# facebookresearch/seamless_communication

Measured on AMD Instinct MI355X. Metric: S2ST utterances/sec (and real-time factor), seamlessM4T_v2_large, 10 s audio, higher is better.
Workload: dtype f32 activations x f16 weights, f32 accumulate

## Files before the change

include/seamless_hip_internal.h:

```cpp
#ifndef SEAMLESS_HIP_INTERNAL_H_
#define SEAMLESS_HIP_INTERNAL_H_

#include "seamless_hip.h"

#ifdef __cplusplus
extern "C" {
#endif

int sc_decoder_step_family(sc_model* m, int rows, int caller);

int sc_op_knob(const char* name, int dflt);

int sc_op_force_general_gemm(int on);
int sc_op_single_plane(int on);
int sc_op_layernorm(const float* d_x, const float* d_gamma, const float* d_beta, float* d_y, int32_t rows, int32_t C,
                    int32_t act);
int sc_op_linear(const float* d_x, const void* d_w_f16, const float* d_bias, const float* d_res, float* d_y,
                 int32_t M, int32_t N, int32_t K, int32_t act, float alpha, int32_t split, int32_t force_gemv);
int sc_op_skinny_linear(const float* d_x, const void* d_w_f16, const float* d_bias, const float* d_res, float* d_y,
                        int32_t M, int32_t N, int32_t K, int32_t act, float alpha);
int sc_op_skinny_res_ln(const float* d_in, const void* d_w_f16, const float* d_bias, float* d_x_inout,
                        const float* d_gamma, const float* d_beta, float* d_h, int32_t M, int32_t N, int32_t K,
                        int32_t splits);
int sc_op_skinny_argmax(const float* d_x, const void* d_w_f16, int32_t M, int32_t N, int32_t K, int32_t step,
// ... 5 lines not shown
int sc_op_dstep_linear_planes(const float* d_x, const void* d_w_f16, const float* d_bias, float* d_y, int32_t M, int32_t N, int32_t K,
                              int32_t act);
int sc_op_dstep_argmax(const float* d_x, const void* d_w_f16, int32_t M, int32_t N, int32_t K, int32_t step,
                       int32_t min_step_for_eos, int32_t force_eos_step, int32_t pad_idx, int32_t eos_idx, int32_t unk_idx,
                       float unk_penalty, int32_t ntl, int32_t* d_idx, float* d_lprob);
int sc_op_dstep_attention(const float* d_proj, int32_t S, const float* d_bias, float* d_kcache, float* d_vcache, int32_t cap,
                          int32_t pos, const int32_t* d_lens, int32_t cross, int32_t nb, int32_t heads, float* d_out);
int sc_op_dstep3_gemv(int32_t mode, const float* d_x, const void* d_w_f16, const float* d_bias, const float* d_gamma,
                      const float* d_beta, const float* d_res, float* d_y, float* d_h, int32_t M, int32_t N, int32_t K, int32_t act,
                      int32_t rg, int32_t shape);
int sc_op_dstep3_argmax(const float* d_x, const void* d_w_f16, int32_t M, int32_t N, int32_t K, int32_t step,
                        int32_t min_step_for_eos, int32_t force_eos_step, int32_t pad_idx, int32_t eos_idx, int32_t unk_idx,
                        float unk_penalty, int32_t* d_idx, float* d_lprob);
int sc_op_chain_bench(int32_t kind, int32_t rows, int32_t n, int32_t reps, float* us_per_kernel);
int sc_op_conv1d(const float* d_x, const void* d_w_f16_packed, const float* d_bias, const float* d_res, float* d_y,
                 int32_t nb, int32_t t_in, int32_t cin, int32_t cout, int32_t k, int32_t stride, int32_t pad,
                 int32_t dil, const int32_t* d_in_lens, int32_t in_act, int32_t act);
int sc_op_pack_conv_weight(const void* d_w_f16, void* d_dst_f16, int32_t cout, int32_t cin, int32_t k);
int sc_op_conv_transpose1d(const float* d_x, const void* d_v_f16, const void* d_g_f16, const float* d_bias,
                           float* d_y, int32_t nb, int32_t t_in, int32_t cin, int32_t cout, int32_t k,
                           int32_t stride, int32_t pad, int32_t in_act);
int sc_op_linear_presplit(const float* d_x, const void* d_w_f16, const float* d_bias, const float* d_res, float* d_y,
                          void* d_yh_f16, void* d_yl_f16, int32_t M, int32_t N, int32_t K, int32_t act, float alpha);
int sc_op_linear_presplit_argmax(const float* d_x, const void* d_w_f16, const float* d_bias, int32_t* d_idx, int32_t M, int32_t N,
                                 int32_t K);
int sc_op_conv1d_presplit(const float* d_x, const void* d_w_f16_packed, const float* d_bias, const float* d_res, float* d_y,
                          void* d_yh_f16, void* d_yl_f16, int32_t nb, int32_t t, int32_t cin, int32_t cout, int32_t k, int32_t pad,
                          int32_t dil, const unsigned char* d_row_valid, int32_t act);
int sc_op_resblock_pair_ps(const float* d_x, const void* d_w1_packed, const float* d_b1, const void* d_w2_packed, const float* d_b2,
                           float* d_out, int32_t nb, int32_t T, int32_t C, int32_t k, int32_t dil);
int sc_op_resblock_pair(const float* d_x, const void* d_w1_packed, const float* d_b1, const void* d_w2_packed,
                        const float* d_b2, float* d_out, int32_t nb, int32_t T, int32_t C, int32_t k, int32_t dil,
                        float slope, const float* d_avg_a, const float* d_avg_b);
int sc_op_mrf_fused(const float* d_x, const void* const* d_w1_packed, const float* const* d_b1, const void* const* d_w2_packed,
                    const float* const* d_b2, float* d_out, int32_t nb, int32_t T, int32_t C, const int32_t* k, const int32_t* dil,
                    float slope);
int sc_op_attention(const float* d_q, const float* d_k, const float* d_v, float* d_out, int32_t nb, int32_t heads,
                    int32_t sq, int32_t skv, int64_t ldq, int64_t ldk, int64_t ldv, int64_t ldo,
                    const int32_t* d_kv_lens, int32_t causal, const float* d_rel_k, int32_t rel_left,
                    int32_t rel_right);
int sc_op_attention_ex(const float* d_q, const float* d_k, const float* d_v, float* d_out, int32_t nb, int32_t heads,
                       int32_t sq, int32_t skv, int64_t ldq, int64_t ldk, int64_t ldv, int64_t ldo,
                       const int32_t* d_kv_lens, int32_t causal, const float* d_rel_k, int32_t rel_left,
                       int32_t rel_right, const int32_t* d_row_off, const float* d_rp_table, int64_t rp_ld,
                       const float* d_q_bias_u, const float* d_q_bias_v, void* d_out_hi, void* d_out_lo, int64_t ldoh);
int sc_op_glu_dwconv(const float* d_x, const float* d_w, float* d_y, int32_t nb, int32_t T, int32_t C, int32_t k,
                     const int32_t* d_lens);
int sc_op_glu_dwconv_ln(const float* d_x, const float* d_w, const float* d_gamma, const float* d_beta, int32_t act, void* d_yh_f16,
                        void* d_yl_f16, int32_t nb, int32_t T, int32_t C, int32_t k, const int32_t* d_lens, int32_t fused);
int sc_op_layernorm2(const float* d_x, const float* d_ga, const float* d_ba, const float* d_gb, const float* d_bb, float* d_y,
                     void* d_yh_f16, void* d_yl_f16, int32_t rows, int32_t C, int32_t fused);
int sc_op_argmax(const float* d_logits, int32_t rows, int32_t V, int32_t* d_idx, float* d_lprob);

#ifdef __cplusplus
}
#endif
#endif
```

seamless_communication_amd/_lib.py:

```python
from __future__ import annotations

import ctypes as C
from pathlib import Path
from typing import Optional

import os

_VARIANT = os.environ.get("SC_LIB_VARIANT", "")
LIB_PATH = Path(__file__).resolve().parent / (f"libseamless_hip.{_VARIANT}.so" if _VARIANT else "libseamless_hip.so")

SC_ABI_VERSION = 9
SC_MAX_UPSAMPLES = 8
SC_MAX_RESBLOCK_KERNELS = 4
SC_MAX_RESBLOCK_DILATIONS = 4
SC_F16, SC_F32, SC_I32 = 0, 1, 2


class SeamlessHipError(RuntimeError):
    pass


class sc_tensor_desc(C.Structure):
    _fields_ = [
        ("name", C.c_char_p),
# ... 106 lines not shown
    "sc_s2st": (C.c_int, [_P, _P, _i, _i, _P, C.POINTER(sc_gen_opts), _P, _i, C.c_float, _P, _P, _P, _i, _P, _P, _i, _P, _P, _P]),
    "sc_prof_enable": (C.c_int, [C.c_int]),
    "sc_prof_reset": (C.c_int, []),
    "sc_prof_report": (C.c_int64, [C.c_char_p, C.c_int64]),
    "sc_text_to_char_seqs": (C.c_int32, [C.c_int32, _P, _P, _P, _P, _P, C.c_int32, C.c_int32, C.c_int32, _P, C.c_int32, C.c_int32,
                                         _P, _P, C.c_int32, _P]),
    "sc_ngram_blocked_tokens": (C.c_int32, [_PI, C.c_int32, C.c_int32, _PI, C.c_int32]),
    "sc_op_knob": (C.c_int, [C.c_char_p, C.c_int]),
    "sc_op_force_general_gemm": (C.c_int, [C.c_int]),
    "sc_op_single_plane": (C.c_int, [C.c_int]),
    "sc_op_layernorm": (C.c_int, [_P, _P, _P, _P, _i, _i, _i]),
    "sc_op_linear": (C.c_int, [_P, _P, _P, _P, _P, _i, _i, _i, _i, C.c_float, _i, _i]),
    "sc_op_skinny_linear": (C.c_int, [_P, _P, _P, _P, _P, _i, _i, _i, _i, C.c_float]),
    "sc_op_skinny_res_ln": (C.c_int, [_P, _P, _P, _P, _P, _P, _P, _i, _i, _i, _i]),
    "sc_op_skinny_argmax": (C.c_int, [_P, _P, _i, _i, _i, _i, _i, _i, _i, _i, _i, C.c_float, _P, _P]),
    "sc_op_dstep_res_ln": (C.c_int, [_P, _P, _P, _P, _P, _P, _P, _i, _i, _i, _i]),
    "sc_op_dstep_linear_planes": (C.c_int, [_P, _P, _P, _P, _i, _i, _i, _i]),
    "sc_op_dstep_argmax": (C.c_int, [_P, _P, _i, _i, _i, _i, _i, _i, _i, _i, _i, C.c_float, _i, _P, _P]),
    "sc_op_resblock_pair_ps": (C.c_int, [_P, _P, _P, _P, _P, _P, _i, _i, _i, _i, _i]),
    "sc_op_glu_dwconv_ln": (C.c_int, [_P, _P, _P, _P, _i, _P, _P, _i, _i, _i, _i, _P, _i]),
    "sc_op_layernorm2": (C.c_int, [_P, _P, _P, _P, _P, _P, _P, _P, _i, _i, _i]),
    "sc_op_dstep3_gemv": (C.c_int, [_i, _P, _P, _P, _P, _P, _P, _P, _P, _i, _i, _i, _i, _i, _i]),
    "sc_op_dstep3_argmax": (C.c_int, [_P, _P, _i, _i, _i, _i, _i, _i, _i, _i, _i, C.c_float, _P, _P]),
    "sc_op_chain_bench": (C.c_int, [_i, _i, _i, _i, _P]),
    "sc_op_dstep_attention": (C.c_int, [_P, _i, _P, _P, _P, _i, _i, _P, _i, _i, _i, _P]),
    "sc_op_conv1d": (C.c_int, [_P, _P, _P, _P, _P, _i, _i, _i, _i, _i, _i, _i, _i, _P, _i, _i]),
    "sc_op_pack_conv_weight": (C.c_int, [_P, _P, _i, _i, _i]),
    "sc_op_conv_transpose1d": (C.c_int, [_P, _P, _P, _P, _P, _i, _i, _i, _i, _i, _i, _i, _i]),
    "sc_op_linear_presplit": (C.c_int, [_P, _P, _P, _P, _P, _P, _P, _i, _i, _i, _i, C.c_float]),
    "sc_op_linear_presplit_argmax": (C.c_int, [_P, _P, _P, _P, _i, _i, _i]),
    "sc_op_conv1d_presplit": (C.c_int, [_P, _P, _P, _P, _P, _P, _P, _i, _i, _i, _i, _i, _i, _i, _P, _i]),
    "sc_op_mrf_fused": (C.c_int, [_P, _P, _P, _P, _P, _P, _i, _i, _i, _P, _P, C.c_float]),
    "sc_op_resblock_pair": (C.c_int, [_P, _P, _P, _P, _P, _P, _i, _i, _i, _i, _i, C.c_float, _P, _P]),
    "sc_op_attention": (C.c_int, [_P, _P, _P, _P, _i, _i, _i, _i, C.c_int64, C.c_int64, C.c_int64, C.c_int64, _P, _i,
                                  _P, _i, _i]),
    "sc_op_attention_ex": (C.c_int, [_P, _P, _P, _P, _i, _i, _i, _i, C.c_int64, C.c_int64, C.c_int64, C.c_int64, _P, _i,
                                     _P, _i, _i, _P, _P, C.c_int64, _P, _P, _P, _P, C.c_int64]),
    "sc_op_glu_dwconv": (C.c_int, [_P, _P, _P, _i, _i, _i, _i, _P]),
    "sc_op_argmax": (C.c_int, [_P, _i, _i, _P, _P]),
}

_lib: Optional[C.CDLL] = None


def load_library() -> C.CDLL:
    global _lib
    if _lib is not None:
        return _lib
    if not LIB_PATH.exists():
        raise SeamlessHipError(
            f"{LIB_PATH} is missing: build it with `python -m seamless_communication_amd.build` "
            "(there is no CPU fallback for the HIP path)"
        )
    lib = C.CDLL(str(LIB_PATH))
    for name, (res, args) in SIGNATURES.items():
        fn = getattr(lib, name)
        fn.restype = res
        fn.argtypes = args
    if lib.sc_abi_version() != SC_ABI_VERSION:
        raise SeamlessHipError(f"ABI mismatch: library {lib.sc_abi_version()} vs binding {SC_ABI_VERSION}")
    _lib = lib
    return lib


def check(status: int, what: str) -> None:
    if status != 0:
# ... 54 lines not shown
```

seamless_communication_amd/build.py:

```python
from __future__ import annotations

import hashlib
import os
import subprocess
import sys
from concurrent.futures import ThreadPoolExecutor
from pathlib import Path

CSRC = Path(__file__).resolve().parent / "csrc"
LIB = Path(__file__).resolve().parent / "libseamless_hip.so"
OBJ_DIR = CSRC / "build"
SOURCES = [
    "common.cpp", "prof.hip", "k_gemm.hip", "k_gemm2.hip", "k_gemm_ps.hip", "k_resblock.hip", "k_skinny.hip", "k_dstep.hip", "k_dstep3.hip", "k_norm.hip", "k_attn.hip", "k_fbank.hip", "k_misc.hip", "k_beam.hip", "k_engine.hip",
    "model_load.hip", "model_encoder.hip", "model_decoder.hip", "model_t2u.hip", "engine.hip", "api.hip",
]
FLAGS = ["--offload-arch=gfx950", "-O3", "-std=c++17", "-fPIC", "-Wall", "-Wno-unused-function"]


def _hipcc() -> str:
    for cand in (os.environ.get("HIPCC"), "/opt/rocm/bin/hipcc", "hipcc"):
        if cand and (os.path.sep not in cand or os.path.exists(cand)):
            return cand
    raise RuntimeError("hipcc not found")


def _stamp(src: Path, flags=FLAGS) -> str:
    h = hashlib.sha256()
    h.update(src.read_bytes())
    for hdr in sorted(CSRC.glob("*.h")) + sorted((CSRC.parent.parent / "include").glob("*.h")):
        h.update(hdr.read_bytes())
    h.update(" ".join(flags).encode())
    return h.hexdigest()


def _compile(src_name: str, verbose: bool, obj_dir: Path = OBJ_DIR, flags=FLAGS) -> Path:
    src = CSRC / src_name
    obj = obj_dir / (src_name + ".o")
    stamp = obj_dir / (src_name + ".stamp")
    digest = _stamp(src, flags)
    if obj.exists() and stamp.exists() and stamp.read_text() == digest:
        return obj
    cmd = [_hipcc(), *flags, "-x", "hip", "-c", str(src), "-o", str(obj)]
    if verbose:
        print(" ".join(cmd), flush=True)
    r = subprocess.run(cmd, capture_output=True, text=True)
    if r.returncode != 0:
# ... 40 lines not shown
```

seamless_communication_amd/csrc/api.hip:

```cpp
#include <atomic>
#include <cstring>
#include <map>
#include <mutex>
#include <set>

#include "../../include/seamless_hip_internal.h"
#include "engine.h"
#include "model.h"

using namespace sc;

struct sc_model {
    Model m;
};

struct sc_engine {
    std::unique_ptr<Engine> e;
    int device = 0;
    const void* weights = nullptr;
    std::set<sc_model*> attached;
};

static std::mutex g_attach_mu;
static std::map<Engine*, sc_engine*> g_engine_owner;
// ... 1162 lines not shown
    conv1d_presplit(tmp, xh, xl, c1, nullptr, nullptr, th, tl, nb, T, (k * dil - dil) / 2, dil, nullptr, ACT_NONE, 0, nullptr, 0.1f, one ? 0 : 1);
    conv1d_presplit(tmp, th, tl, c2, d_x, d_out, nullptr, nullptr, nb, T, (k - 1) / 2, 1, nullptr, ACT_NONE, 0, nullptr, 0.1f, one ? 0 : 1);
    SC_HIP(hipStreamSynchronize(g_op_stream));
    SC_API_END
}

int sc_op_resblock_pair(const float* d_x, const void* d_w1_packed, const float* d_b1, const void* d_w2_packed,
                        const float* d_b2, float* d_out, int32_t nb, int32_t T, int32_t C, int32_t k, int32_t dil,
                        float slope, const float* d_avg_a, const float* d_avg_b) {
    SC_API_BEGIN
    SC_CHECK(d_x && d_w1_packed && d_w2_packed && d_out, "sc_op_resblock_pair: null argument");
    ResPairArgs a;
    a.x = d_x;
    a.out = d_out;
    a.w1 = static_cast<const __half*>(d_w1_packed);
    a.w2 = static_cast<const __half*>(d_w2_packed);
    a.ldw1 = a.ldw2 = align_up((int64_t)C * k, 32);
    a.b1 = d_b1;
    a.b2 = d_b2;
    a.nb = nb;
    a.T = T;
    a.C = C;
    a.k = k;
    a.dil = dil;
    a.slope = slope;
    a.avg_a = d_avg_a;
    a.avg_b = d_avg_b;
    a.single = g_op_single.load();
    launch_resblock_pair(a, g_op_stream);
    SC_HIP(hipStreamSynchronize(g_op_stream));
    SC_API_END
}

int sc_op_mrf_fused(const float* d_x, const void* const* d_w1_packed, const float* const* d_b1, const void* const* d_w2_packed,
                    const float* const* d_b2, float* d_out, int32_t nb, int32_t T, int32_t C, const int32_t* k, const int32_t* dil,
                    float slope) {
    SC_API_BEGIN
    SC_CHECK(d_x && d_w1_packed && d_b1 && d_w2_packed && d_b2 && d_out && k && dil, "sc_op_mrf_fused: null argument");
    MrfArgs a;
    a.x = d_x;
    a.out = d_out;
    a.nb = nb;
    a.T = T;
    a.C = C;
    a.slope = slope;
    for (int j = 0; j < 3; ++j) a.k[j] = k[j];
    for (int q = 0; q < 9; ++q) {
        a.dil[q] = dil[q];
        a.w1[q] = static_cast<const __half*>(d_w1_packed[q]);
        a.w2[q] = static_cast<const __half*>(d_w2_packed[q]);
        a.ldw1[q] = a.ldw2[q] = align_up((int64_t)C * k[q / 3], 32);
        a.b1[q] = d_b1[q];
        a.b2[q] = d_b2[q];
    }
    a.single = g_op_single.load();
    launch_mrf_fused(a, g_op_stream);
    SC_HIP(hipStreamSynchronize(g_op_stream));
    SC_API_END
}

int sc_op_attention(const float* d_q, const float* d_k, const float* d_v, float* d_out, int32_t nb, int32_t heads,
                    int32_t sq, int32_t skv, int64_t ldq, int64_t ldk, int64_t ldv, int64_t ldo, const int32_t* d_kv_lens,
                    int32_t causal, const float* d_rel_k, int32_t rel_left, int32_t rel_right) {
    SC_API_BEGIN
    AttnArgs a;
    a.q = d_q;
// ... 110 lines not shown
```

seamless_communication_amd/csrc/common.cpp:

```cpp
#include "common.h"
#include <cstdlib>
#include <cstring>

namespace sc {

static thread_local char g_err[1024] = "";

void set_error(const char* fmt, ...) {
    va_list ap;
    va_start(ap, fmt);
    vsnprintf(g_err, sizeof(g_err), fmt, ap);
    va_end(ap);
}

const char* get_error() { return g_err; }

namespace knob {
namespace {
struct Knob {
    const char* name;
    int kind;
    const char* what;
};
const Knob knob_table[] = {
    {"SC_DEBUG_NUMERICS", 0, "honour the switches that change results"},
    {"SC_DEBUG_FILL", 0, "fill fresh scratch blocks with NaN (tests)"},
    {"SC_SPLIT_MODE", 1, "1: Conformer products on the hi fp16 plane only (precision study)"},
    {"SC_ATTN_F32", 1, "attention on the exact-fp32 matrix instruction (round 1)"},
    {"SC_ATTN_VALU", 1, "attention on the vector ALU (round 1)"},
    {"SC_DECODER_GEN1", 1, "decoder step on the first-generation kernels"},
    {"SC_DECODER_GEN2", 1, "decoder step on the second-generation chain"},
    {"SC_DECODE_STEPWISE", 1, "teacher-forced pass step by step instead of one batched forward"},
    {"SC_VOC_SPLIT", 1, "vocoder ResBlock products on both fp16 planes of their activations again (bit 0 wide stages, bit 2 narrow stages); default: hi plane only"},
    {"SC_GEMM_GENERAL", 0, "general GEMM kernel instead of the fast path"}, {"SC_GEMM_PF2", 0, "GEMM prefetch depth"},
    {"SC_GEMM_GROUP_M", 0, "GEMM workgroup order"}, {"SC_GEMM_TILE", 0, "GEMM tile override"},
    {"SC_PS_ILV", 0, "DMA GEMM: interleaved issue"}, {"SC_PS_HALF", 0, "DMA GEMM: mid-slab barrier"}, {"SC_PS_PP", 0, "0: 8-wave DMA GEMM in lock step instead of alternating load / compute segments"},
    {"SC_PS_TILE", 0, "DMA GEMM: largest tile"}, {"SC_PS_MIN256", 0, "DMA GEMM: tiles needed for 256 x 256"},
    {"SC_PS_MIN128", 0, "DMA GEMM: tiles needed for 128 x 128"},
    {"SC_PRESPLIT", 0, "0: Conformer operands split on the fly"}, {"SC_ENC_FUSE", 0, "0: separate Conformer element-wise launches"},
    {"SC_D3_RG_SMALL", 0, "decoder step: rows per row group, N = 1024 products"}, {"SC_D3_RG_FFN", 0, "decoder step: rows per row group, FFN-in"},
    {"SC_G3_STATIONARY", 0, "row-group products of wide steps: 0 one workgroup per row group, n = workgroup budget of the weight-stationary launch"},
    {"SC_G3_TILES", 0, "0: FFN-out of wide steps on the weight-stationary row-group walk instead of tile-owning waves"},
    {"SC_G3_TOUCH", 0, "weight-stationary products: bit 0 cooperative L2 touch of the activations, bit 1 K slices per XCD (FFN-out); default 3"},
    {"SC_D3_FFN_IN", 0, "decoder step: FFN-in workgroup shape"}, {"SC_D3_FFN_OUT", 0, "decoder step: FFN-out workgroup shape"},
    {"SC_MMA_GRAPH", 0, "streaming decoder step from a captured graph"}, 
    {"SC_T2U_GROUPS", 0, "NAR T2U: length buckets"}, {"SC_T2U_PACKED", 0, "0: NAR decoder on padded buckets"},
    {"SC_T2U_FUSED_ARGMAX", 0, "0: unit logits written out, arg-max as its own launch"},
    {"SC_VOC_PS", 0, "0: vocoder wide stages on the register-staged convolution"}, {"SC_VOC_MRF", 0, "0: narrow vocoder stages as nine pair launches"},
    {"SC_VOC_GROUPS", 0, "vocoder: length buckets"}, {"SC_VOC_GROUP_OVERHEAD", 0, "vocoder: bucket planning overhead rows"},
    {"SC_VOC_STREAMS", 0, "vocoder: side chains"},
    {"SC_ENGINE_RG_SMALL", 0, "decode engine: rows per row group, N = 1024 products"},
    {"SC_BEAM_COMPACT", 2, "0: beam search keeps finished utterances' slots"},
    {"SC_GREEDY_COMPACT", 2, "0: greedy generation keeps finished rows in their slots"}, {"SC_GREEDY_POLL", 2, "steps between looks at the finished flags"},
};
constexpr int N_KNOBS = sizeof(knob_table) / sizeof(knob_table[0]);
struct State {
    bool set[N_KNOBS];
    int val[N_KNOBS];
    bool numerics = false;
};
const State& state() {
    static const State st = [] {
        State s{};
        const char* dn = getenv("SC_DEBUG_NUMERICS");
        s.numerics = dn && atoi(dn) != 0;
        for (int i = 0; i < N_KNOBS; ++i) {
// ... 53 lines not shown
```

seamless_communication_amd/csrc/kernels.h:

```cpp
#pragma once
#include <atomic>

#include "common.h"
#include "prof.h"

namespace sc {

enum Act { ACT_NONE = 0, ACT_RELU = 1, ACT_SILU = 2, ACT_TANH = 3 };
enum InAct { IN_NONE = 0, IN_LRELU_01 = 1, IN_LRELU_001 = 2 };

struct GemmArgs {
    const float* A = nullptr;
    int64_t lda = 0;
    const __half* W = nullptr;
    int64_t ldw = 0;
    int64_t w_phase_stride = 0;
    const float* bias = nullptr;
    const float* res = nullptr;
    int64_t ldr = 0;
    float* C = nullptr;
    int64_t ldc = 0;
    int M = 0;
    int N = 0;
    int K = 0;
// ... 32 lines not shown
    int64_t ldcs = 0;
    int M = 0, N = 0, K = 0;
    int act = ACT_NONE;
    float alpha = 1.0f;
    int split = 1;
    float plane_neg_slope = 1.0f;
    int conv_taps = 0, conv_cin = 0, conv_dil = 1, conv_pad = 0, rows_per_item = 0;
    const unsigned char* row_valid = nullptr;
    const int2* row_pos = nullptr;
    float2* amax = nullptr;
    int amax_ld = 0;
};
void launch_gemm_presplit(const GemmPsArgs& a, hipStream_t s);
int gemm_presplit_amax_chunks(int M, int N);
void launch_amax_finish(const float2* part, int ld, int rows, int* out_idx, hipStream_t s);

struct ResPairArgs {
    const float* x = nullptr;
    float* out = nullptr;
    const __half* w1 = nullptr;
    int64_t ldw1 = 0;
    const float* b1 = nullptr;
    const __half* w2 = nullptr;
    int64_t ldw2 = 0;
    const float* b2 = nullptr;
    int nb = 0, T = 0, C = 0, k = 0, dil = 1;
    float slope = 0.1f;
    const float* avg_a = nullptr;
    const float* avg_b = nullptr;
    int single = 0;
};
bool resblock_pair_supported(int C, int k, int dil);
void launch_resblock_pair(const ResPairArgs& a, hipStream_t s);

struct MrfArgs {
    const float* x = nullptr;
    float* out = nullptr;
    int nb = 0, T = 0, C = 0;
    float slope = 0.1f;
    int halo = 0;
    int k[3] = {0, 0, 0};
    int dil[9] = {1, 1, 1, 1, 1, 1, 1, 1, 1};
    const __half* w1[9] = {};
    const __half* w2[9] = {};
    int64_t ldw1[9] = {};
    int64_t ldw2[9] = {};
    const float* b1[9] = {};
    const float* b2[9] = {};
    int single = 0;
};
bool mrf_fused_supported(int C, const int* k, const int* dil);
void launch_mrf_fused(const MrfArgs& a, hipStream_t s);

void launch_gemv(const float* x, int64_t ldx, const __half* W, int64_t ldw, const float* bias,
                 const float* res, int64_t ldr, float* out, int64_t ldo, int M, int N, int K,
                 int act, float alpha, hipStream_t s);

struct SkinnyArgs {
    const float* A = nullptr;
    int64_t lda = 0;
    const __half* W = nullptr;
    int64_t ldw = 0;
    const float* bias = nullptr;
    const float* res = nullptr;
    int64_t ldr = 0;
    float* C = nullptr;
// ... 396 lines not shown
```

seamless_communication_amd/csrc/model_t2u.hip:

```cpp
#include <cstdlib>

#include "model.h"

namespace sc {

namespace {

void attention_self(Model& m, const float* qkv, int M, float* out, int nb, int S, const int* d_lens) {
    AttnArgs a;
    a.q = qkv;
    a.k = qkv + M;
    a.v = qkv + 2 * M;
    a.out = out;
    a.ldq = a.ldk = a.ldv = 3 * M;
    a.ldo = M;
    a.nb = nb;
    a.heads = m.cfg.num_heads;
    a.Sq = S;
    a.Skv = S;
    a.kv_lens = d_lens;
    launch_attention(a, m.stream);
}

void text_to_char_seqs(const Model& m, const int32_t* text_seqs, int n, int s_text, std::vector<int32_t>& char_lens,
// ... 449 lines not shown
    int ch = c.voc_upsample_initial_channel;
    int t = T;
    Buf<float> x;
    {
        Buf<float> in(m.pp(), (size_t)n * T * (E + Lg + Sp));
        launch_vocoder_embed(d_units, n, T, m.voc_dict, E, m.voc_lang, Lg, d_lang, m.voc_spkr, Sp, d_spkr, in, m.stream);
        x = Buf<float>(m.pp(), (size_t)n * T * ch);
        conv1d(m, in, m.voc_pre, nullptr, x, n, T, 1, 3, 1, nullptr, IN_NONE, ACT_NONE);
    }
    const int nk = c.voc_num_resblock_kernels;
    SC_CHECK(nk == 3, "sc_vocode: %d resblock kernels (only 3 is implemented)", nk);
    static const int voc_split = knob::value("SC_VOC_SPLIT", 0);
    const int voc_single = (voc_split & 1 ? 0 : 1) | (voc_split & 4 ? 0 : 4);
    for (int i = 0; i < c.voc_num_upsamples; ++i) {
        const ConvT& up = m.voc_ups[i];
        const int t2 = t * up.stride;
        ch = up.cout;
        const size_t sz = (size_t)n * t2 * ch;
        Buf<float> y(m.pp(), sz), tmp(m.pp(), sz), ra(m.pp(), sz), rb(m.pp(), sz);
        Buf<float> rout[3] = {Buf<float>(m.pp(), sz), Buf<float>(m.pp(), sz), Buf<float>(m.pp(), sz)};
        conv_transpose1d(m, x, up, y, n, t, IN_LRELU_01);
        bool fused_avg = false;
        x = Buf<float>(m.pp(), sz);
        static const bool voc_ps = knob::value("SC_VOC_PS", 1) != 0;
        bool wide_ps = voc_ps && g_force_general_gemm.load(std::memory_order_relaxed) == 0 && ch >= 128 && ch % 32 == 0 &&
                       (int64_t)n * t2 * ch * 2 < (1ll << 31);
        for (int j = 0; j < nk && wide_ps; ++j) {
            const ResBlock& r = m.voc_res[i * nk + j];
            for (size_t d = 0; d < r.dil.size(); ++d)
                wide_ps = wide_ps && r.convs1[d].cin == ch && r.convs1[d].cout == ch && r.convs2[d].cin == ch && r.convs2[d].cout == ch &&
                          r.convs1[d].kpad == ch * r.convs1[d].k && r.convs2[d].kpad == ch * r.convs2[d].k && (r.convs1[d].k & 1) &&
                          (r.convs2[d].k & 1);
        }
        if (wide_ps) {
            const bool one_plane = (voc_single & 1) != 0;
            Buf<__half> planes(m.pp(), (one_plane ? 3 : 6) * sz);
            __half* py_h = planes.get();
            __half* pt_h = py_h + sz;
            __half* pn_h = pt_h + sz;
            __half* py_l = one_plane ? nullptr : pn_h + sz;
            __half* pt_l = one_plane ? nullptr : py_l + sz;
            __half* pn_l = one_plane ? nullptr : pt_l + sz;
            launch_lrelu_split_f32(y, 0.1f, py_h, py_l, (int64_t)sz, m.stream);
            for (int j = 0; j < nk; ++j) {
                const ResBlock& r = m.voc_res[i * nk + j];
                const float* cur = y;
                const __half *ch_ = py_h, *cl_ = py_l;
                const int nd = (int)r.dil.size();
                for (int d = 0; d < nd; ++d) {
                    const int k = r.convs1[d].k, k2 = r.convs2[d].k;
                    const bool last = d == nd - 1;
                    float* dst = last ? rout[j].get() : ((d & 1) ? rb.get() : ra.get());
                    const int split = one_plane ? 0 : 1;
                    conv1d_presplit(m, ch_, cl_, r.convs1[d], nullptr, nullptr, pt_h, pt_l, n, t2, (k * r.dil[d] - r.dil[d]) / 2, r.dil[d], nullptr,
                                    ACT_NONE, 0, nullptr, 0.1f, split);
                    conv1d_presplit(m, pt_h, pt_l, r.convs2[d], cur, dst, last ? nullptr : pn_h, last ? nullptr : pn_l, n, t2, (k2 - 1) / 2, 1,
                                    nullptr, ACT_NONE, 0, nullptr, 0.1f, split);
                    cur = dst;
                    ch_ = pn_h;
                    cl_ = pn_l;
                }
            }
            launch_avg3(rout[0], rout[1], rout[2], x, (int64_t)sz, m.stream);
            t = t2;
            continue;
        }
        static const bool voc_mrf = knob::value("SC_VOC_MRF", 1) != 0;
// ... 3 lines not shown
            for (int j = 0; j < nk && ok; ++j) {
                const ResBlock& r = m.voc_res[i * nk + j];
                ok = r.dil.size() == 3;
                for (int d = 0; d < 3 && ok; ++d) {
                    const Conv &c1 = r.convs1[d], &c2 = r.convs2[d];
                    ok = c1.k == r.convs1[0].k && c2.k == c1.k && c1.cin == ch && c1.cout == ch && c2.cin == ch && c2.cout == ch;
                    const int q = j * 3 + d;
                    a.dil[q] = r.dil[d];
                    a.w1[q] = c1.w, a.ldw1[q] = c1.kpad, a.b1[q] = c1.b;
                    a.w2[q] = c2.w, a.ldw2[q] = c2.kpad, a.b2[q] = c2.b;
                }
                if (ok) a.k[j] = r.convs1[0].k;
            }
            if (ok && mrf_fused_supported(ch, a.k, a.dil)) {
                a.x = y.get();
                a.out = x.get();
                a.nb = n;
                a.T = t2;
                a.C = ch;
                a.slope = 0.1f;
                a.single = (voc_single & 4) ? 1 : 0;
                launch_mrf_fused(a, m.stream);
                t = t2;
                continue;
            }
        }
        for (int j = 0; j < nk; ++j) {
            const ResBlock& r = m.voc_res[i * nk + j];
            const float* cur = y;
            const int nd = (int)r.dil.size();
            for (int d = 0; d < nd; ++d) {
                const int k = r.convs1[d].k;
                float* dst = (d == nd - 1) ? rout[j].get() : ((d & 1) ? rb.get() : ra.get());
                const bool fuse = g_force_general_gemm.load(std::memory_order_relaxed) == 0 && r.convs2[d].k == k &&
                                  r.convs1[d].cin == ch && r.convs1[d].cout == ch && r.convs2[d].cin == ch &&
                                  r.convs2[d].cout == ch && resblock_pair_supported(ch, k, r.dil[d]);
                if (fuse) {
                    ResPairArgs a;
                    a.x = cur;
                    a.w1 = r.convs1[d].w;
                    a.ldw1 = r.convs1[d].kpad;
                    a.b1 = r.convs1[d].b;
                    a.w2 = r.convs2[d].w;
                    a.ldw2 = r.convs2[d].kpad;
                    a.b2 = r.convs2[d].b;
                    a.nb = n;
                    a.T = t2;
                    a.C = ch;
                    a.k = k;
                    a.dil = r.dil[d];
                    a.slope = 0.1f;
                    a.single = (voc_single & 4) ? 1 : 0;
                    if (j == nk - 1 && d == nd - 1) {
                        a.avg_a = rout[0];
                        a.avg_b = rout[1];
                        dst = x.get();
                        fused_avg = true;
                    }
                    a.out = dst;
                    launch_resblock_pair(a, m.stream);
                } else {
                    conv1d(m, cur, r.convs1[d], nullptr, tmp, n, t2, 1, (k * r.dil[d] - r.dil[d]) / 2, r.dil[d], nullptr,
                           IN_LRELU_01, ACT_NONE);
                    conv1d(m, tmp, r.convs2[d], cur, dst, n, t2, 1, (k - 1) / 2, 1, nullptr, IN_LRELU_01, ACT_NONE);
                }
                cur = dst;
            }
        }
        if (!fused_avg) launch_avg3(rout[0], rout[1], rout[2], x, (int64_t)sz, m.stream);
        t = t2;
    }
    conv1d(m, x, m.voc_post, nullptr, d_wav, n, t, 1, 3, 1, nullptr, IN_LRELU_001, ACT_TANH);
}

int vocoder_halo_units(const Model& m) {
    const sc_config& c = m.cfg;
    double halo = 3.0, rate = 1.0;
    for (int i = 0; i < c.voc_num_upsamples; ++i) {
        const ConvT& up = m.voc_ups[i];
        halo += (double)up.taps / rate;
        rate *= up.stride;
        int widest = 0;
        for (int j = 0; j < c.voc_num_resblock_kernels; ++j) {
            const ResBlock& r = m.voc_res[i * c.voc_num_resblock_kernels + j];
            int reach = 0;
            for (size_t d = 0; d < r.dil.size(); ++d) reach += (r.convs1[d].k - 1) * r.dil[d] / 2 + (r.convs2[d].k - 1) / 2;
            widest = std::max(widest, reach);
        }
        halo += (double)widest / rate;
    }
    halo += 3.0 / rate;
    return (int)halo + 8;
}
// ... 123 lines not shown
```

Measured before the change: 328.1.

## Fuse wide vocoder ResBlock dilation pairs into one DMA-fed MFMA kernel

Adds a kernel for vocoder ResBlock stages with C=128 or 256 that runs both convolutions of a dilation pair in one launch. The input tile with halo is staged as fp16 in LDS, weights stream through a three-stage LDS ring via buffer_load-to-LDS, and the intermediate activation stays in LDS. The final residual add and the three-way branch average are applied in the epilogue. This replaces two DMA GEMM launches per pair plus the fp16 plane splitting, removing the global round trip of the intermediate, at the cost of halo recompute and heavy LDS use that limits occupancy.

```diff
diff --git a/include/seamless_hip_internal.h b/include/seamless_hip_internal.h
--- a/include/seamless_hip_internal.h
+++ b/include/seamless_hip_internal.h
@@ -61,6 +61,9 @@
 int sc_op_resblock_pair(const float* d_x, const void* d_w1_packed, const float* d_b1, const void* d_w2_packed,
                         const float* d_b2, float* d_out, int32_t nb, int32_t T, int32_t C, int32_t k, int32_t dil,
                         float slope, const float* d_avg_a, const float* d_avg_b);
+int sc_op_resblock_pair_wide(const float* d_x, const void* d_w1_packed, const float* d_b1, const void* d_w2_packed, const float* d_b2,
+                             float* d_out, const float* d_avg_a, const float* d_avg_b, int32_t nb, int32_t T, int32_t C, int32_t k,
+                             int32_t dil);
 int sc_op_mrf_fused(const float* d_x, const void* const* d_w1_packed, const float* const* d_b1, const void* const* d_w2_packed,
                     const float* const* d_b2, float* d_out, int32_t nb, int32_t T, int32_t C, const int32_t* k, const int32_t* dil,
                     float slope);
diff --git a/seamless_communication_amd/_lib.py b/seamless_communication_amd/_lib.py
--- a/seamless_communication_amd/_lib.py
+++ b/seamless_communication_amd/_lib.py
@@ -162,6 +162,7 @@
     "sc_op_conv1d_presplit": (C.c_int, [_P, _P, _P, _P, _P, _P, _P, _i, _i, _i, _i, _i, _i, _i, _P, _i]),
     "sc_op_mrf_fused": (C.c_int, [_P, _P, _P, _P, _P, _P, _i, _i, _i, _P, _P, C.c_float]),
     "sc_op_resblock_pair": (C.c_int, [_P, _P, _P, _P, _P, _P, _i, _i, _i, _i, _i, C.c_float, _P, _P]),
+    "sc_op_resblock_pair_wide": (C.c_int, [_P, _P, _P, _P, _P, _P, _P, _P, _i, _i, _i, _i, _i]),
     "sc_op_attention": (C.c_int, [_P, _P, _P, _P, _i, _i, _i, _i, C.c_int64, C.c_int64, C.c_int64, C.c_int64, _P, _i,
                                   _P, _i, _i]),
     "sc_op_attention_ex": (C.c_int, [_P, _P, _P, _P, _i, _i, _i, _i, C.c_int64, C.c_int64, C.c_int64, C.c_int64, _P, _i,
diff --git a/seamless_communication_amd/build.py b/seamless_communication_amd/build.py
--- a/seamless_communication_amd/build.py
+++ b/seamless_communication_amd/build.py
@@ -11,7 +11,7 @@
 LIB = Path(__file__).resolve().parent / "libseamless_hip.so"
 OBJ_DIR = CSRC / "build"
 SOURCES = [
-    "common.cpp", "prof.hip", "k_gemm.hip", "k_gemm2.hip", "k_gemm_ps.hip", "k_resblock.hip", "k_skinny.hip", "k_dstep.hip", "k_dstep3.hip", "k_norm.hip", "k_attn.hip", "k_fbank.hip", "k_misc.hip", "k_beam.hip", "k_engine.hip",
+    "common.cpp", "prof.hip", "k_gemm.hip", "k_gemm2.hip", "k_gemm_ps.hip", "k_resblock.hip", "k_resblock_wide.hip", "k_skinny.hip", "k_dstep.hip", "k_dstep3.hip", "k_norm.hip", "k_attn.hip", "k_fbank.hip", "k_misc.hip", "k_beam.hip", "k_engine.hip",
     "model_load.hip", "model_encoder.hip", "model_decoder.hip", "model_t2u.hip", "engine.hip", "api.hip",
 ]
 FLAGS = ["--offload-arch=gfx950", "-O3", "-std=c++17", "-fPIC", "-Wall", "-Wno-unused-function"]
diff --git a/seamless_communication_amd/csrc/api.hip b/seamless_communication_amd/csrc/api.hip
--- a/seamless_communication_amd/csrc/api.hip
+++ b/seamless_communication_amd/csrc/api.hip
@@ -1218,6 +1218,33 @@
     SC_API_END
 }
 
+int sc_op_resblock_pair_wide(const float* d_x, const void* d_w1_packed, const float* d_b1, const void* d_w2_packed, const float* d_b2,
+                             float* d_out, const float* d_avg_a, const float* d_avg_b, int32_t nb, int32_t T, int32_t C, int32_t k,
+                             int32_t dil) {
+    SC_API_BEGIN
+    SC_CHECK(d_x && d_w1_packed && d_w2_packed && d_out, "sc_op_resblock_pair_wide: null argument");
+    ResPairArgs a;
+    a.x = d_x;
+    a.out = d_out;
+    a.w1 = static_cast<const __half*>(d_w1_packed);
+    a.w2 = static_cast<const __half*>(d_w2_packed);
+    a.ldw1 = a.ldw2 = (int64_t)C * k;
+    a.b1 = d_b1;
+    a.b2 = d_b2;
+    a.nb = nb;
+    a.T = T;
+    a.C = C;
+    a.k = k;
+    a.dil = dil;
+    a.slope = 0.1f;
+    a.avg_a = d_avg_a;
+    a.avg_b = d_avg_b;
+    a.single = 1;
+    launch_resblock_wide(a, g_op_stream);
+    SC_HIP(hipStreamSynchronize(g_op_stream));
+    SC_API_END
+}
+
 int sc_op_mrf_fused(const float* d_x, const void* const* d_w1_packed, const float* const* d_b1, const void* const* d_w2_packed,
                     const float* const* d_b2, float* d_out, int32_t nb, int32_t T, int32_t C, const int32_t* k, const int32_t* dil,
                     float slope) {
diff --git a/seamless_communication_amd/csrc/common.cpp b/seamless_communication_amd/csrc/common.cpp
--- a/seamless_communication_amd/csrc/common.cpp
+++ b/seamless_communication_amd/csrc/common.cpp
@@ -32,6 +32,7 @@
     {"SC_DECODER_GEN2", 1, "decoder step on the second-generation chain"},
     {"SC_DECODE_STEPWISE", 1, "teacher-forced pass step by step instead of one batched forward"},
     {"SC_VOC_SPLIT", 1, "vocoder ResBlock products on both fp16 planes of their activations again (bit 0 wide stages, bit 2 narrow stages); default: hi plane only"},
+    {"SC_VOC_WIDE_PAIR", 1, "0: wide vocoder stages (C = 128 / 256) as two DMA GEMM launches per dilation pair instead of one fused pair kernel"},
     {"SC_GEMM_GENERAL", 0, "general GEMM kernel instead of the fast path"}, {"SC_GEMM_PF2", 0, "GEMM prefetch depth"},
     {"SC_GEMM_GROUP_M", 0, "GEMM workgroup order"}, {"SC_GEMM_TILE", 0, "GEMM tile override"},
     {"SC_PS_ILV", 0, "DMA GEMM: interleaved issue"}, {"SC_PS_HALF", 0, "DMA GEMM: mid-slab barrier"}, {"SC_PS_PP", 0, "0: 8-wave DMA GEMM in lock step instead of alternating load / compute segments"},
diff --git a/seamless_communication_amd/csrc/k_resblock_wide.hip b/seamless_communication_amd/csrc/k_resblock_wide.hip
--- /dev/null
+++ b/seamless_communication_amd/csrc/k_resblock_wide.hip
@@ -0,0 +1,277 @@
+#include <algorithm>
+
+#include "kernels.h"
+
+namespace sc {
+
+namespace {
+
+typedef _Float16 half8_t __attribute__((ext_vector_type(8)));
+typedef _Float16 half4_t __attribute__((ext_vector_type(4)));
+typedef float float16_t __attribute__((ext_vector_type(16)));
+typedef float f32x4_t __attribute__((ext_vector_type(4)));
+typedef int i32x4_t __attribute__((ext_vector_type(4)));
+
+constexpr int RW_M1 = 128;
+constexpr int RW_BK = 32;
+constexpr int RW_STAGES = 3;
+constexpr int RW_LDS_MAX = 160 * 1024;
+#define RW_LDS_PTR(p) ((__attribute__((address_space(3))) void*)(p))
+
+template <int C>
+struct RwCfg {
+    static constexpr int NWAVE = C / 32;
+    static constexpr int WGN = NWAVE / 2;
+    static constexpr int BCH = C / (16 * NWAVE);
+    static_assert(C == 128 || C == 256, "wide pair kernel: C = 128 or 256");
+    static_assert(BCH == 2, "two DMA chunks per wave and slab");
+};
+
+__device__ __forceinline__ float rw_lrelu(float v, float slope) { return fmaxf(v, 0.f) + slope * fminf(v, 0.f); }
+
+__device__ __forceinline__ i32x4_t rw_rsrc(const void* base, uint32_t bytes) {
+    const uint64_t b = reinterpret_cast<uint64_t>(base);
+    i32x4_t r;
+    r[0] = __builtin_amdgcn_readfirstlane((int)(uint32_t)b);
+    r[1] = __builtin_amdgcn_readfirstlane((int)(uint32_t)((b >> 32) & 0xffff));
+    r[2] = __builtin_amdgcn_readfirstlane((int)bytes);
+    r[3] = 0x00020000;
+    return r;
+}
+
+__device__ __forceinline__ int rw_swz(int row, int s) { return row * 64 + ((s ^ ((row >> 2) & 3)) << 4); }
+
+template <int C>
+__global__ __launch_bounds__(C * 2) void resblock_wide_kernel(ResPairArgs p, int tiles, uint32_t w1_bytes, uint32_t w2_bytes) {
+    using Cfg = RwCfg<C>;
+    constexpr int NT = Cfg::NWAVE * 64;
+    constexpr int CS = C + 8;
+    constexpr int VPR = C / 4;
+    constexpr int SLAB_HALFS = C * RW_BK;
+    constexpr int BCH = Cfg::BCH;
+    extern __shared__ __attribute__((aligned(16))) unsigned char rw_smem[];
+    _Float16* const ring = reinterpret_cast<_Float16*>(rw_smem);
+    _Float16* const xs = ring + RW_STAGES * SLAB_HALFS;
+
+    const int k = p.k, dil = p.dil, T = p.T;
+    const int H2 = (k - 1) / 2, H1 = dil * (k - 1) / 2;
+    const int TT = RW_M1 - 2 * H2;
+    const int R0 = RW_M1 + 2 * H1;
+    const int NS = k * C / RW_BK;
+    const int NSL = 2 * NS;
+    const float slope = p.slope;
+
+    const int tid = threadIdx.x, lane = tid & 63;
+    const int wave = __builtin_amdgcn_readfirstlane(tid >> 6);
+    const int wm = wave / Cfg::WGN, wn = wave % Cfg::WGN;
+    const int n = blockIdx.x / tiles;
+    const int t0 = (blockIdx.x - n * tiles) * TT;
+    const float* __restrict__ xn = p.x + (int64_t)n * T * C;
+
+    const i32x4_t rw1 = rw_rsrc(p.w1, w1_bytes);
+    const i32x4_t rw2 = rw_rsrc(p.w2, w2_bytes);
+    uint32_t b_voff1[BCH], b_voff2[BCH];
+#pragma unroll
+    for (int j = 0; j < BCH; ++j) {
+        const int row = 16 * (wave * BCH + j) + (lane >> 2);
+        const int seg = (lane & 3) ^ ((row >> 2) & 3);
+        b_voff1[j] = (uint32_t)((row * p.ldw1 + seg * 8) * 2);
+        b_voff2[j] = (uint32_t)((row * p.ldw2 + seg * 8) * 2);
+    }
+    auto issue = [&](int h) {
+        const bool second = h >= NS;
+        const int soff = (second ? h - NS : h) * (RW_BK * 2);
+        _Float16* const st = ring + (h % RW_STAGES) * SLAB_HALFS;
+#pragma unroll
+        for (int j = 0; j < BCH; ++j) {
+            const uint32_t voff = second ? b_voff2[j] : b_voff1[j];
+            const uint32_t m0 = __builtin_amdgcn_readfirstlane((int)(uint32_t)(uintptr_t)RW_LDS_PTR(st + (wave * BCH + j) * 512));
+            if (second)
+                asm volatile("s_mov_b32 m0, %0\n\tbuffer_load_dwordx4 %1, %2, %3 offen lds" : : "s"(m0), "v"(voff), "s"(rw2), "s"(soff) : "memory");
+            else
+                asm volatile("s_mov_b32 m0, %0\n\tbuffer_load_dwordx4 %1, %2, %3 offen lds" : : "s"(m0), "v"(voff), "s"(rw1), "s"(soff) : "memory");
+        }
+    };
+
+    issue(0);
+    if (NSL > 1) issue(1);
+    float bias1[2], bias2[2];
+#pragma unroll
+    for (int j = 0; j < 2; ++j) {
+        const int col = wn * 64 + j * 32 + (lane & 31);
+        bias1[j] = p.b1 ? p.b1[col] : 0.f;
+        bias2[j] = p.b2 ? p.b2[col] : 0.f;
+    }
+    {
+        constexpr int U = 8;
+        const int total = R0 * VPR;
+        for (int base = tid; base < total; base += NT * U) {
+            f32x4_t v[U];
+#pragma unroll
+            for (int u = 0; u < U; ++u) {
+                const int i = base + u * NT;
+                const int r = i / VPR, c4 = i - r * VPR;
+                const int t = t0 - H2 - H1 + r;
+                v[u] = f32x4_t{0.f, 0.f, 0.f, 0.f};
+                if (i < total && t >= 0 && t < T) v[u] = *reinterpret_cast<const f32x4_t*>(xn + (int64_t)t * C + c4 * 4);
+            }
+#pragma unroll
+            for (int u = 0; u < U; ++u) {
+                const int i = base + u * NT;
+                if (i >= total) continue;
+                const int r = i / VPR, c4 = i - r * VPR;
+#pragma unroll
+                for (int e = 0; e < 4; ++e) v[u][e] = rw_lrelu(v[u][e], slope);
+                *reinterpret_cast<half4_t*>(xs + r * CS + c4 * 4) = __builtin_convertvector(v[u], half4_t);
+            }
+        }
+    }
+    __builtin_amdgcn_s_waitcnt(0x0070);
+
+    const int koff = (lane >> 5) * 8;
+    int a_row[2], b_off[2][2];
+#pragma unroll
+    for (int i = 0; i < 2; ++i) a_row[i] = 64 * wm + 32 * i + (lane & 31);
+#pragma unroll
+    for (int kc = 0; kc < 2; ++kc)
+#pragma unroll
+        for (int j = 0; j < 2; ++j) b_off[j][kc] = rw_swz(wn * 64 + j * 32 + (lane & 31), kc * 2 + (lane >> 5));
+
+    float16_t acc[2][2];
+#pragma unroll
+    for (int i = 0; i < 2; ++i)
+#pragma unroll
+        for (int j = 0; j < 2; ++j)
+#pragma unroll
+            for (int r = 0; r < 16; ++r) acc[i][j][r] = 0.f;
+
+    auto step = [&](int g, int tap_step) {
+        if (g + 1 < NSL) __builtin_amdgcn_s_waitcnt(0x0072);
+        else __builtin_amdgcn_s_waitcnt(0x0070);
+        __builtin_amdgcn_s_barrier();
+        asm volatile("" ::: "memory");
+        const int kk = (g < NS ? g : g - NS) * RW_BK;
+        const int tap = kk / C, c0 = kk - tap * C;
+        const char* const st = reinterpret_cast<const char*>(ring + (g % RW_STAGES) * SLAB_HALFS);
+        half8_t af[2][2], bf[2][2];
+#pragma unroll
+        for (int kc = 0; kc < 2; ++kc) {
+#pragma unroll
+            for (int i = 0; i < 2; ++i)
+                af[kc][i] = *reinterpret_cast<const half8_t*>(xs + (a_row[i] + tap * tap_step) * CS + c0 + kc * 16 + koff);
+#pragma unroll
+            for (int j = 0; j < 2; ++j) bf[kc][j] = *reinterpret_cast<const half8_t*>(st + b_off[j][kc]);
+        }
+        const bool more = g + 2 < NSL;
+        __builtin_amdgcn_sched_barrier(0);
+#pragma unroll
+        for (int kc = 0; kc < 2; ++kc)
+#pragma unroll
+            for (int i = 0; i < 2; ++i)
+#pragma unroll
+                for (int j = 0; j < 2; ++j) {
+                    acc[i][j] = __builtin_amdgcn_mfma_f32_32x32x16_f16(af[kc][i], bf[kc][j], acc[i][j], 0, 0, 0);
+                    if (kc == 0 && i == 0 && j == 1) {
+                        __builtin_amdgcn_sched_barrier(0);
+                        if (more) issue(g + 2);
+                        __builtin_amdgcn_sched_barrier(0);
+                    }
+                }
+        asm volatile("" ::: "memory");
+    };
+
+    for (int g = 0; g < NS; ++g) step(g, dil);
+    __builtin_amdgcn_s_waitcnt(0xC07F);
+    __builtin_amdgcn_s_barrier();
+    asm volatile("" ::: "memory");
+#pragma unroll
+    for (int i = 0; i < 2; ++i)
+#pragma unroll
+        for (int j = 0; j < 2; ++j) {
+            const int col = wn * 64 + j * 32 + (lane & 31);
+#pragma unroll
+            for (int r = 0; r < 16; ++r) {
+                const int row = 64 * wm + 32 * i + (r & 3) + 8 * (r >> 2) + 4 * (lane >> 5);
+                const int t = t0 - H2 + row;
+                const float v = (t >= 0 && t < T) ? rw_lrelu((acc[i][j][r] + bias1[j]) * 1.0f, slope) : 0.f;
+                xs[row * CS + col] = (_Float16)v;
+                acc[i][j][r] = 0.f;
+            }
+        }
+
+    for (int g = NS; g < NSL; ++g) step(g, 1);
+
+    float* __restrict__ outn = p.out + (int64_t)n * T * C;
+    const int64_t nTC = (int64_t)n * T * C;
+#pragma unroll
+    for (int i = 0; i < 2; ++i)
+#pragma unroll
+        for (int j = 0; j < 2; ++j) {
+            const int col = wn * 64 + j * 32 + (lane & 31);
+            float res[16], va[16], vb[16];
+#pragma unroll
+            for (int r = 0; r < 16; ++r) {
+                const int row = 64 * wm + 32 * i + (r & 3) + 8 * (r >> 2) + 4 * (lane >> 5);
+                const int64_t off = (int64_t)min(t0 + row, T - 1) * C + col;
+                res[r] = xn[off];
+                if (p.avg_a) {
+                    va[r] = p.avg_a[nTC + off];
+                    vb[r] = p.avg_b[nTC + off];
+                }
+            }
+#pragma unroll
+            for (int r = 0; r < 16; ++r) {
+                const int row = 64 * wm + 32 * i + (r & 3) + 8 * (r >> 2) + 4 * (lane >> 5);
+                const int t = t0 + row;
+                float v = (acc[i][j][r] + bias2[j]) * 1.0f + res[r];
+                if (p.avg_a) v = ((va[r] + vb[r]) + v) / 3.0f;
+                if (row < TT && t < T) outn[(int64_t)t * C + col] = v;
+            }
+        }
+}
+
+size_t rw_lds_bytes(int C, int k, int dil) {
+    return (size_t)RW_STAGES * C * RW_BK * sizeof(_Float16) + (size_t)(RW_M1 + dil * (k - 1)) * (C + 8) * sizeof(_Float16);
+}
+
+template <int C>
+void launch_rw_cfg(const ResPairArgs& a, hipStream_t s) {
+    static bool attr_set = false;
+    if (!attr_set) {
+        SC_HIP(hipFuncSetAttribute(reinterpret_cast<const void*>(&resblock_wide_kernel<C>), hipFuncAttributeMaxDynamicSharedMemorySize, RW_LDS_MAX));
+        attr_set = true;
+    }
+    const int TT = RW_M1 - (a.k - 1);
+    const int tiles = cdiv(a.T, TT);
+    const size_t lds = rw_lds_bytes(C, a.k, a.dil);
+    char name[48];
+    snprintf(name, sizeof(name), "resblock_wide_c%d", C);
+    const double rows = (double)a.nb * a.T;
+    prof::Scope scope(name, 2.0 * 2.0 * rows * C * (double)C * a.k,
+                      4.0 * rows * C * (a.avg_a ? 4.0 : 2.0) + 2.0 * 2.0 * C * (double)C * a.k, s);
+    hipLaunchKernelGGL((resblock_wide_kernel<C>), dim3((unsigned)(a.nb * tiles)), dim3(RwCfg<C>::NWAVE * 64), lds, s, a, tiles,
+                       (uint32_t)(C * a.ldw1 * 2), (uint32_t)(C * a.ldw2 * 2));
+}
+
+}
+
+bool resblock_wide_supported(int C, int k, int dil) {
+    if (!(C == 128 || C == 256) || k < 1 || (k & 1) == 0 || dil < 1) return false;
+    return RW_M1 - (k - 1) >= 32 && rw_lds_bytes(C, k, dil) <= (size_t)RW_LDS_MAX;
+}
+
+void launch_resblock_wide(const ResPairArgs& a, hipStream_t s) {
+    SC_CHECK(resblock_wide_supported(a.C, a.k, a.dil), "resblock wide pair: unsupported C=%d k=%d dil=%d", a.C, a.k, a.dil);
+    SC_CHECK(a.single, "resblock wide pair: multiplies the hi fp16 plane only");
+    SC_CHECK(a.nb > 0 && a.T > 0 && a.x && a.out && a.w1 && a.w2 && a.x != a.out, "resblock wide pair: empty problem, null operand or in-place call");
+    SC_CHECK(a.ldw1 % 8 == 0 && a.ldw2 % 8 == 0 && a.ldw1 >= (int64_t)a.k * a.C && a.ldw2 >= (int64_t)a.k * a.C &&
+                 (int64_t)a.C * std::max(a.ldw1, a.ldw2) * 2 < (1ll << 31),
+             "resblock wide pair: packed weight rows too short or too long");
+    SC_CHECK((a.avg_a == nullptr) == (a.avg_b == nullptr), "resblock wide pair: avg_a/avg_b must be given together");
+    SC_CHECK((int64_t)a.nb * cdiv(a.T, RW_M1 - (a.k - 1)) < (1ll << 31), "resblock wide pair: grid too large");
+    if (a.C == 128) launch_rw_cfg<128>(a, s);
+    else launch_rw_cfg<256>(a, s);
+    SC_LAUNCH_CHECK();
+}
+
+}
diff --git a/seamless_communication_amd/csrc/kernels.h b/seamless_communication_amd/csrc/kernels.h
--- a/seamless_communication_amd/csrc/kernels.h
+++ b/seamless_communication_amd/csrc/kernels.h
@@ -88,6 +88,8 @@
 };
 bool resblock_pair_supported(int C, int k, int dil);
 void launch_resblock_pair(const ResPairArgs& a, hipStream_t s);
+bool resblock_wide_supported(int C, int k, int dil);
+void launch_resblock_wide(const ResPairArgs& a, hipStream_t s);
 
 struct MrfArgs {
     const float* x = nullptr;
diff --git a/seamless_communication_amd/csrc/model_t2u.hip b/seamless_communication_amd/csrc/model_t2u.hip
--- a/seamless_communication_amd/csrc/model_t2u.hip
+++ b/seamless_communication_amd/csrc/model_t2u.hip
@@ -505,7 +505,15 @@
                           r.convs1[d].kpad == ch * r.convs1[d].k && r.convs2[d].kpad == ch * r.convs2[d].k && (r.convs1[d].k & 1) &&
                           (r.convs2[d].k & 1);
         }
-        if (wide_ps) {
+        static const bool voc_wide_pair = knob::value("SC_VOC_WIDE_PAIR", 1) != 0;
+        bool wide_pair = voc_wide_pair && (voc_single & 1) && g_force_general_gemm.load(std::memory_order_relaxed) == 0;
+        for (int j = 0; j < nk && wide_pair; ++j) {
+            const ResBlock& r = m.voc_res[i * nk + j];
+            for (size_t d = 0; d < r.dil.size(); ++d)
+                wide_pair = wide_pair && r.convs1[d].cin == ch && r.convs1[d].cout == ch && r.convs2[d].cin == ch && r.convs2[d].cout == ch &&
+                            r.convs2[d].k == r.convs1[d].k && resblock_wide_supported(ch, r.convs1[d].k, r.dil[d]);
+        }
+        if (wide_ps && !wide_pair) {
             const bool one_plane = (voc_single & 1) != 0;
             Buf<__half> planes(m.pp(), (one_plane ? 3 : 6) * sz);
             __half* py_h = planes.get();
@@ -575,9 +583,9 @@
             for (int d = 0; d < nd; ++d) {
                 const int k = r.convs1[d].k;
                 float* dst = (d == nd - 1) ? rout[j].get() : ((d & 1) ? rb.get() : ra.get());
-                const bool fuse = g_force_general_gemm.load(std::memory_order_relaxed) == 0 && r.convs2[d].k == k &&
-                                  r.convs1[d].cin == ch && r.convs1[d].cout == ch && r.convs2[d].cin == ch &&
-                                  r.convs2[d].cout == ch && resblock_pair_supported(ch, k, r.dil[d]);
+                const bool fuse = wide_pair || (g_force_general_gemm.load(std::memory_order_relaxed) == 0 && r.convs2[d].k == k &&
+                                                r.convs1[d].cin == ch && r.convs1[d].cout == ch && r.convs2[d].cin == ch &&
+                                                r.convs2[d].cout == ch && resblock_pair_supported(ch, k, r.dil[d]));
                 if (fuse) {
                     ResPairArgs a;
                     a.x = cur;
@@ -593,7 +601,7 @@
                     a.k = k;
                     a.dil = r.dil[d];
                     a.slope = 0.1f;
-                    a.single = (voc_single & 4) ? 1 : 0;
+                    a.single = wide_pair ? 1 : (voc_single & 4) ? 1 : 0;
                     if (j == nk - 1 && d == nd - 1) {
                         a.avg_a = rout[0];
                         a.avg_b = rout[1];
@@ -601,7 +609,8 @@
                         fused_avg = true;
                     }
                     a.out = dst;
-                    launch_resblock_pair(a, m.stream);
+                    if (wide_pair) launch_resblock_wide(a, m.stream);
+                    else launch_resblock_pair(a, m.stream);
                 } else {
                     conv1d(m, cur, r.convs1[d], nullptr, tmp, n, t2, 1, (k * r.dil[d] - r.dil[d]) / 2, r.dil[d], nullptr,
                            IN_LRELU_01, ACT_NONE);
```

Result: no change. 331.4, median of 6 (+1.0%).
